# eromero-vlc/superbblas

Hardware: AMD Instinct MI355X
Metric: lattice contraction GFLOP/s + permute GB/s, 16^4 spin×color, 1/2/4/8 GPUs (higher is better)
Workload: dtype complex<f64>

## Files before the change

superbblas_amd/csrc/capi.cpp:

```cpp
#include "plan.h"
#include <atomic>
#include <algorithm>
#include <functional>
#include <memory>
#include <unordered_map>

#include <rccl/rccl.h>

#include <cstdlib>
#include <cstring>
#include <mutex>

namespace sbx {
BsrOp *bsr_create(int nd, int ni, int dtype, const std::vector<std::vector<Range>> &pi,
                  const Coor &dimi, const std::vector<std::vector<Range>> &pd, const Coor &dimd,
                  const Coor &blocki, const Coor &blockd, bool block_im_fast,
                  const std::vector<const int *> &ii, const std::vector<const int *> &jj,
                  const std::vector<const void *> &v, const std::vector<int> &devs, bool reverse_jj,
                  const Comm &comm, const Coor *kroni = nullptr, const Coor *krond = nullptr,
                  const std::vector<const void *> *kronv = nullptr);
void bsr_destroy(BsrOp *op);
void bsr_krylov(const BsrOp &op, const Scalar &alpha, const std::string &oi,
                const std::string &od, const DistTensor &x, const Coor &fromx, const Coor &sizex,
                const Scalar &beta, const DistTensor &y, const Coor &fromy, const Coor &sizey,
// ... 304 lines not shown
        tapes().clear();
    });
}

int sbx_clear_handles(void) {
    return guard([&] {
        trim_pools();
        destroy_streams();
    });
}

int sbx_allocate(unsigned long long bytes, sbx_context ctx, void **ptr) {
    return guard([&] {
        if (ctx.plat == SBX_GPU) {
            *ptr = device_alloc(bytes, ctx.device);
        } else {
            SBX_HIP_CHECK(hipHostMalloc(ptr, bytes, hipHostMallocDefault));
        }
    });
}

int sbx_deallocate(void *ptr, sbx_context ctx) {
    return guard([&] {
        if (!ptr) return;
        if (ctx.plat == SBX_GPU) {
            set_device(ctx.device);
            SBX_HIP_CHECK(hipStreamSynchronize(get_stream(ctx.device)));
            device_free(ptr, ctx.device);
        } else {
            SBX_HIP_CHECK(hipHostFree(ptr));
        }
    });
}

int sbx_set_custom_allocator(sbx_alloc_fn alloc, sbx_free_fn dealloc, void *user) {
    return guard([&] {
        if ((alloc == nullptr) != (dealloc == nullptr))
            throw Error("set_custom_allocator: give both functions or neither");
        set_alloc_hooks(alloc, dealloc, user);
    });
}

int sbx_allocate_from_cache(unsigned long long bytes, sbx_context ctx, void **ptr) {
    return guard([&] {
        if (ctx.plat != SBX_GPU) throw Error("allocate_from_cache: GPU contexts only");
        *ptr = scratch_alloc(bytes, ctx.device);
    });
}

int sbx_release_to_cache(void *ptr, sbx_context ctx) {
    return guard([&] {
        if (ctx.plat != SBX_GPU) throw Error("release_to_cache: GPU contexts only");
        scratch_free(ptr, ctx.device);
    });
}

int sbx_cache_usage(int device, unsigned long long *cached, unsigned long long *live) {
    return guard([&] {
        std::size_t c = 0, l = 0;
        cache_usage(device, &c, &l);
        if (cached) *cached = c;
        if (live) *live = l;
    });
}

int sbx_tune_set(const char *key, long long value) {
    return guard([&] {
        if (!key) throw Error("tune_set: null key");
        const std::string k(key);
        if (k == "copy.budget") g_copy_tune.budget = (long)value;
        else if (k == "copy.run") g_copy_tune.run = (long)value;
        else if (k == "copy.nt") g_copy_tune.nt = (int)value;
        else if (k == "copy.max_elems") g_copy_tune.max_elems = (long)value;
        else if (k == "copy.pair") g_copy_tune.pair = (int)value;
        else if (k == "copy.order") g_copy_tune.order = (int)value;
        else if (k == "copy.trans") g_copy_tune.trans = (int)value;
        else if (k == "copy.btrans") g_copy_tune.btrans = (int)value;
        else if (k == "gemm.max_bytes") g_gemm_tune.max_bytes = (long)value;
        else if (k == "gemm.loaders") g_gemm_tune.loaders = (int)value;
        else if (k == "gemm.dma_spread") g_gemm_tune.dma_spread = (int)value;
        else if (k == "gemm.dma_nt") g_gemm_tune.dma_nt = (int)value;
        else if (k == "gemm.lean") g_gemm_tune.lean = (int)value;
        else if (k == "gemm.skinny") g_gemm_tune.skinny = (int)value;
        else if (k == "bsr.variant") g_bsr_tune.variant = (int)value;
        else if (k == "bsr.row_max_cols") g_bsr_tune.row_max_cols = (long)value;
        else if (k == "bsr.split_max_cols") g_bsr_tune.split_max_cols = (long)value;
        else if (k == "bsr.split_cw") g_bsr_tune.split_cw = (int)value;
        else if (k == "bsr.split_jb") g_bsr_tune.split_jb = (int)value;
        else if (k == "bsr.split_ilv") g_bsr_tune.split_ilv = (int)value;
        else if (k == "bsr.kron_mfma") g_bsr_tune.kron_mfma = (int)value;
        else if (k == "bsr.kron_mfma_min_cols") g_bsr_tune.kron_mfma_min_cols = (long)value;
        else if (k == "bsr.kron_pack") g_bsr_tune.kron_pack = (int)value;
        else if (k == "bsr.kron_xlds") g_bsr_tune.kron_xlds = (int)value;
        else if (k == "bsr.kron_ylds") g_bsr_tune.kron_ylds = (int)value;
        else if (k == "bsr.kron_spin") g_bsr_tune.kron_spin = (int)value;
        else if (k == "bsr.kron_adj") g_bsr_tune.kron_adj = (int)value;
        else if (k == "bsr.kron_spin_min_cols") g_bsr_tune.kron_spin_min_cols = (long)value;
        else if (k == "bsr.kron_order") g_bsr_tune.kron_order = (int)value;
        else if (k == "bsr.nt") g_bsr_tune.nt = (int)value;
        else if (k == "dense.wave") g_dense_wave = (int)value;
        else if (k == "bsr.blk_pd") g_bsr_tune.blk_pd = (int)value;
        else if (k == "bsr.blk_mfma") g_bsr_tune.blk_mfma = (int)value;
        else if (k == "bsr.blk_min") g_bsr_tune.blk_min = (int)value;
        else if (k == "bsr.mixed") g_bsr_tune.mixed = (int)value;
        else if (k == "bsr.mixed12_min_cols") g_bsr_tune.mixed12_min_cols = (long)value;
        else if (k == "bsr.mixed12_pack") g_bsr_tune.mixed12_pack = (int)value;
        else if (k == "bsr.adj_inplace") g_bsr_tune.adj_inplace = (int)value;
        else if (k == "bsr.kron_mixed") g_bsr_tune.kron_mixed = (int)value;
        else if (k == "bsr.adj_copy_bytes") throw Error("tune_set: bsr.adj_copy_bytes is read-only");
        else if (k == "bsr.tile") g_bsr_tune.tile = (int)value;
        else if (k == "bsr.tile_min_cols") g_bsr_tune.tile_min_cols = value;
        else if (k == "gemm.m3") g_gemm_tune.m3 = (int)value;
        else if (k == "gemm.splits") g_gemm_tune.splits = (int)value;
        else if (k == "gemm.t48") g_gemm_tune.t48 = (int)value;
        else if (k == "gemm.share_ab") g_gemm_tune.share_ab = (int)value;
        else if (k == "gemm.herm") g_gemm_tune.herm = (int)value;
        else if (k == "gemm.frag") g_gemm_tune.frag = (int)value;
        else if (k == "gemm.dot_wgs") g_gemm_tune.dot_wgs = (int)value;
        else if (k == "gemm.frag_tall") g_gemm_tune.frag_tall = (int)value;
        else if (k == "gemm.frag_pair") g_gemm_tune.frag_pair = (int)value;
        else if (k == "gemm.frag_nt") g_gemm_tune.frag_nt = (int)value;
        else if (k == "gemm.frag_small") g_gemm_tune.frag_small = (int)value;
        else if (k == "gemm.frag_uk") g_gemm_tune.frag_uk = (int)value;
        else if (k == "gemm.frag_waves") g_gemm_tune.frag_waves = (int)value;
        else if (k == "gemm.clock") {
            g_gemm_tune.clock = (int)value;
            unsigned long long v[3];
            gemm_clock_read(current_device(), v, true);
        }
        else if (k == "dist.reduce") g_dist_reduce = (int)value;
        else if (k == "debug.level") g_debug_level = (int)value;
        else if (k == "debug.corrupt_copy") g_debug_corrupt = (int)value;
        else if (k == "dist.reduce_calls") g_dist_reduce_calls = value;
        else if (k == "dist.force_peer") g_dist_force_peer = (int)value;
        else if (k == "dist.peer_copies") g_dist_peer_copies = value;
        else if (k.compare(0, 6, "alloc.") == 0) alloc_tune(key, nullptr, &value);
        else throw Error("tune_set: unknown key " + k);
        if (k.compare(0, 5, "copy.") == 0) {
            std::lock_guard<std::mutex> g(g_tape_mutex);
            tapes().clear();
        }
    });
}

int sbx_tune_get(const char *key, long long *value) {
    return guard([&] {
        if (!key || !value) throw Error("tune_get: null argument");
        const std::string k(key);
        if (k == "copy.budget") *value = g_copy_tune.budget;
        else if (k == "copy.run") *value = g_copy_tune.run;
        else if (k == "copy.nt") *value = g_copy_tune.nt;
        else if (k == "copy.max_elems") *value = g_copy_tune.max_elems;
        else if (k == "copy.pair") *value = g_copy_tune.pair;
        else if (k == "copy.order") *value = g_copy_tune.order;
        else if (k == "copy.trans") *value = g_copy_tune.trans;
        else if (k == "copy.btrans") *value = g_copy_tune.btrans;
        else if (k == "copy.last_pair") *value = g_copy_tune.last_pair;
        else if (k == "gemm.max_bytes") *value = g_gemm_tune.max_bytes;
        else if (k == "gemm.loaders") *value = g_gemm_tune.loaders;
        else if (k == "gemm.dma_spread") *value = g_gemm_tune.dma_spread;
        else if (k == "gemm.dma_nt") *value = g_gemm_tune.dma_nt;
        else if (k == "gemm.lean") *value = g_gemm_tune.lean;
        else if (k == "gemm.last_lean") *value = g_gemm_tune.last_lean;
        else if (k == "gemm.skinny") *value = g_gemm_tune.skinny;
        else if (k == "bsr.variant") *value = g_bsr_tune.variant;
        else if (k == "bsr.row_max_cols") *value = g_bsr_tune.row_max_cols;
        else if (k == "bsr.split_max_cols") *value = g_bsr_tune.split_max_cols;
        else if (k == "bsr.split_cw") *value = g_bsr_tune.split_cw;
        else if (k == "bsr.split_jb") *value = g_bsr_tune.split_jb;
        else if (k == "bsr.split_ilv") *value = g_bsr_tune.split_ilv;
        else if (k == "bsr.kron_mfma") *value = g_bsr_tune.kron_mfma;
        else if (k == "bsr.kron_mfma_min_cols") *value = g_bsr_tune.kron_mfma_min_cols;
        else if (k == "bsr.kron_pack") *value = g_bsr_tune.kron_pack;
        else if (k == "bsr.kron_xlds") *value = g_bsr_tune.kron_xlds;
        else if (k == "bsr.kron_ylds") *value = g_bsr_tune.kron_ylds;
        else if (k == "bsr.kron_spin") *value = g_bsr_tune.kron_spin;
        else if (k == "bsr.kron_adj") *value = g_bsr_tune.kron_adj;
        else if (k == "bsr.kron_spin_min_cols") *value = g_bsr_tune.kron_spin_min_cols;
        else if (k == "bsr.kron_order") *value = g_bsr_tune.kron_order;
        else if (k == "bsr.nt") *value = g_bsr_tune.nt;
        else if (k == "dense.wave") *value = g_dense_wave;
        else if (k == "bsr.blk_pd") *value = g_bsr_tune.blk_pd;
        else if (k == "bsr.blk_mfma") *value = g_bsr_tune.blk_mfma;
        else if (k == "bsr.blk_min") *value = g_bsr_tune.blk_min;
        else if (k == "bsr.tile") *value = g_bsr_tune.tile;
        else if (k == "bsr.tile_min_cols") *value = g_bsr_tune.tile_min_cols;
        else if (k == "bsr.mixed") *value = g_bsr_tune.mixed;
        else if (k == "bsr.mixed12_min_cols") *value = g_bsr_tune.mixed12_min_cols;
        else if (k == "bsr.mixed12_pack") *value = g_bsr_tune.mixed12_pack;
        else if (k == "bsr.last_kernel") *value = g_bsr_tune.last;
        else if (k == "bsr.last_mixed") *value = g_bsr_tune.last_mixed;
        else if (k == "bsr.adj_inplace") *value = g_bsr_tune.adj_inplace;
        else if (k == "bsr.kron_mixed") *value = g_bsr_tune.kron_mixed;
        else if (k == "bsr.adj_copy_bytes") *value = g_bsr_tune.adj_copy_bytes;
        else if (k == "gemm.m3") *value = g_gemm_tune.m3;
        else if (k == "gemm.splits") *value = g_gemm_tune.splits;
        else if (k == "gemm.t48") *value = g_gemm_tune.t48;
        else if (k == "gemm.share_ab") *value = g_gemm_tune.share_ab;
        else if (k == "gemm.herm") *value = g_gemm_tune.herm;
        else if (k == "gemm.last_herm") *value = g_gemm_tune.last_herm;
        else if (k == "gemm.frag") *value = g_gemm_tune.frag;
        else if (k == "gemm.dot_wgs") *value = g_gemm_tune.dot_wgs;
        else if (k == "gemm.frag_tall") *value = g_gemm_tune.frag_tall;
        else if (k == "gemm.frag_pair") *value = g_gemm_tune.frag_pair;
        else if (k == "gemm.frag_nt") *value = g_gemm_tune.frag_nt;
        else if (k == "gemm.frag_small") *value = g_gemm_tune.frag_small;
        else if (k == "gemm.frag_uk") *value = g_gemm_tune.frag_uk;
        else if (k == "gemm.frag_waves") *value = g_gemm_tune.frag_waves;
        else if (k == "gemm.clock") *value = g_gemm_tune.clock;
        else if (k == "gemm.clock_cycles" || k == "gemm.clock_ticks" || k == "gemm.clock_launches") {
            unsigned long long v[3];
            gemm_clock_read(current_device(), v, false);
            *value = (long long)v[k == "gemm.clock_cycles" ? 0 : k == "gemm.clock_ticks" ? 1 : 2];
        }
        else if (k == "dist.reduce") *value = g_dist_reduce;
        else if (k == "debug.level") *value = g_debug_level;
        else if (k == "debug.corrupt_copy") *value = g_debug_corrupt;
        else if (k == "dist.reduce_calls") *value = g_dist_reduce_calls;
        else if (k == "dist.force_peer") *value = g_dist_force_peer;
        else if (k == "dist.peer_copies") *value = g_dist_peer_copies;
        else if (k == "detail.last_device") *value = g_detail_last_device;
        else if (k.compare(0, 6, "alloc.") == 0) alloc_tune(key, value, nullptr);
        else throw Error("tune_get: unknown key " + k);
    });
}

int sbx_timings_enable(int on) {
    return guard([&] { timings_enable(on != 0); });
}

int sbx_timings_filter(const char *names) {
    return guard([&] { timings_filter(names && *names ? names : nullptr); });
}

int sbx_timings_reset(void) {
    return guard([&] { timings_reset(); });
}

int sbx_timings_get(const char *name, double *ms, long long *calls) {
    return guard([&] {
        if (!name || !ms || !calls) throw Error("timings_get: null argument");
        timings_get(name, ms, calls);
    });
}

int sbx_timings_report(char *buf, int len) {
    return guard([&] {
// ... 1023 lines not shown
```

superbblas_amd/csrc/kernels_gemm.hip:

```cpp
#include "sbx_internal.h"

#include <algorithm>
#include <map>
#include <mutex>
#include <cstdint>
#include <type_traits>

namespace sbx {
GemmTune g_gemm_tune;
namespace {

template <typename R> struct Mfma;
template <> struct Mfma<double> {
    typedef double acc_t __attribute__((ext_vector_type(4)));
    static __device__ __forceinline__ acc_t mma(double a, double b, acc_t c) {
        return __builtin_amdgcn_mfma_f64_16x16x4f64(a, b, c, 0, 0, 0);
    }
    static __device__ __forceinline__ int row(int lane, int r) { return (lane >> 4) + 4 * r; }
};
template <> struct Mfma<float> {
    typedef float acc_t __attribute__((ext_vector_type(4)));
    static __device__ __forceinline__ acc_t mma(float a, float b, acc_t c) {
        return __builtin_amdgcn_mfma_f32_16x16x4f32(a, b, c, 0, 0, 0);
    }
    static __device__ __forceinline__ int row(int lane, int r) { return ((lane >> 4) << 2) + r; }
};

template <typename R, bool CPLX> struct Elem;
template <> struct Elem<double, true> { typedef double2 type; };
template <> struct Elem<double, false> { typedef double type; };
template <> struct Elem<float, true> { typedef float2 type; };
template <> struct Elem<float, false> { typedef float type; };

template <typename E> __device__ __forceinline__ E zero_elem() { return E{}; }
[[maybe_unused]] __device__ __forceinline__ double2 conj_if(double2 v, bool c) { return c ? double2{v.x, -v.y} : v; }
__device__ __forceinline__ float2 conj_if(float2 v, bool c) { return c ? float2{v.x, -v.y} : v; }
__device__ __forceinline__ double conj_if(double v, bool) { return v; }
__device__ __forceinline__ float conj_if(float v, bool) { return v; }

template <typename E> __device__ __forceinline__ E buf_load(__amdgpu_buffer_rsrc_t r, unsigned off);
template <> [[maybe_unused]] __device__ __forceinline__ double2 buf_load<double2>(__amdgpu_buffer_rsrc_t r, unsigned off) {
    auto v = __builtin_amdgcn_raw_buffer_load_b128(r, off, 0, 0);
    return __builtin_bit_cast(double2, v);
}
template <> __device__ __forceinline__ double buf_load<double>(__amdgpu_buffer_rsrc_t r, unsigned off) {
    auto v = __builtin_amdgcn_raw_buffer_load_b64(r, off, 0, 0);
    return __builtin_bit_cast(double, v);
}
template <> __device__ __forceinline__ float2 buf_load<float2>(__amdgpu_buffer_rsrc_t r, unsigned off) {
    auto v = __builtin_amdgcn_raw_buffer_load_b64(r, off, 0, 0);
    return __builtin_bit_cast(float2, v);
}
template <> __device__ __forceinline__ float buf_load<float>(__amdgpu_buffer_rsrc_t r, unsigned off) {
    auto v = __builtin_amdgcn_raw_buffer_load_b32(r, off, 0, 0);
    return __builtin_bit_cast(float, v);
}

struct GemmKArgs {
    long m, n, k, batch;
    const void *a;
    long sa_m, sa_k, sa_b;
    const void *b;
    long sb_k, sb_n, sb_b;
    void *c;
    long sc_m, sc_n, sc_b;
    double alpha_re, alpha_im, beta_re, beta_im;
    int conja, conjb;
    int splits;
    int herm;
    long kchunk;
    void *work;
    unsigned long long *probe;
    int probe_all;
    int tm, tn;
    unsigned a_bytes, b_bytes;
    int split;
    long m_lo, n_lo, k_lo;
    long sa_m_hi, sa_k_hi, sb_k_hi, sb_n_hi, sc_m_hi, sc_n_hi;
    int same_ab;
    int dma_nt;
    int pair_a, pair_b;
};

__device__ __forceinline__ long split_off(long i, long lo, long s, long s_hi) {
    const unsigned q = (unsigned)i / (unsigned)lo;
    return (long)q * s_hi + (long)((unsigned)i - q * (unsigned)lo) * s;
}
__device__ __forceinline__ long c_off(const GemmKArgs &p, long gi, long gj) {
    return p.split ? split_off(gi, p.m_lo, p.sc_m, p.sc_m_hi) + split_off(gj, p.n_lo, p.sc_n, p.sc_n_hi)
                   : gi * p.sc_m + gj * p.sc_n;
}

template <typename R>
__device__ __forceinline__ void epilogue_store(R *cptr, R vr, R vi, const GemmKArgs &p, bool cplx) {
    if (cplx) {
        R ar = (R)p.alpha_re, ai = (R)p.alpha_im;
        R outr = ar * vr - ai * vi, outi = ar * vi + ai * vr;
        if (p.beta_re != 0 || p.beta_im != 0) {
            R br = (R)p.beta_re, bi = (R)p.beta_im;
            R cr = cptr[0], ci = cptr[1];
            outr += br * cr - bi * ci;
            outi += br * ci + bi * cr;
        }
        cptr[0] = outr;
        cptr[1] = outi;
    } else {
        R out = (R)p.alpha_re * vr;
        if (p.beta_re != 0) out += (R)p.beta_re * cptr[0];
        cptr[0] = out;
    }
}


__device__ __forceinline__ int xcd_workgroup() {
    const int nwg = gridDim.x, bid = blockIdx.x;
    const int xcd = bid & 7, q = nwg >> 3, rr = nwg & 7;
    return (xcd < rr ? xcd * (q + 1) : rr * (q + 1) + (xcd - rr) * q) + (bid >> 3);
}

struct KRange {
    long begin, end;
};
__device__ __forceinline__ KRange split_k_range(const GemmKArgs &p, int split) {
    const long k_begin = (long)split * p.kchunk;
    return KRange{k_begin, min(p.k, k_begin + p.kchunk)};
}

struct Tile {
    int ti, tj, split;
    long bb, m0, n0, k_begin, k_end;
    __device__ __forceinline__ void finish(const GemmKArgs &p, int rest, int BM, int BN) {
        split = rest % p.splits;
        bb = rest / p.splits;
        m0 = (long)ti * BM, n0 = (long)tj * BN;
        const KRange kr = split_k_range(p, split);
        k_begin = kr.begin, k_end = kr.end;
    }
};
__device__ __forceinline__ Tile tile_of(const GemmKArgs &p, int wg, int BM, int BN) {
    Tile t;
    t.ti = wg % p.tm;
    int rest = wg / p.tm;
    t.tj = rest % p.tn;
    t.finish(p, rest / p.tn, BM, BN);
    return t;
}
__device__ __forceinline__ Tile upper_tile_of(const GemmKArgs &p, int wg, int BM) {
    Tile t;
    const long ntri = (long)p.tm * (p.tm + 1) / 2;
    const long tt = wg % ntri;
    long c = (long)((__fsqrt_rn(8.f * (float)tt + 1.f) - 1.f) * 0.5f);
    while (c * (c + 1) / 2 > tt) --c;
    while ((c + 1) * (c + 2) / 2 <= tt) ++c;
    t.tj = (int)c;
    t.ti = (int)(tt - c * (c + 1) / 2);
    t.finish(p, (int)(wg / ntri), BM, BM);
    return t;
}

template <typename E>
__device__ __forceinline__ __amdgpu_buffer_rsrc_t operand_rsrc(const void *base, long bb, long s_b,
                                                               unsigned bytes) {
    return __builtin_amdgcn_make_buffer_rsrc((void *)((const E *)base + bb * s_b), (short)0,
                                             (int)bytes, 0x00020000);
}

template <typename R> struct ConjMask {
    typedef typename std::conditional<sizeof(R) == 8, unsigned long long, unsigned>::type U;
    U ma, mb;
    __device__ __forceinline__ ConjMask(const GemmKArgs &p) {
        const U sign = (U)1 << (sizeof(R) * 8 - 1);
        ma = p.conja ? sign : 0, mb = p.conjb ? sign : 0;
    }
    static __device__ __forceinline__ R flip(R v, U m) {
        return __builtin_bit_cast(R, __builtin_bit_cast(U, v) ^ m);
    }
    template <typename E, int MT, int NT>
    __device__ __forceinline__ void apply(E (&af)[MT], E (&bf)[NT]) const {
#pragma unroll
        for (int i = 0; i < MT; ++i) af[i].y = flip(af[i].y, ma);
#pragma unroll
        for (int j = 0; j < NT; ++j) bf[j].y = flip(bf[j].y, mb);
    }
};

template <typename A, int MT, int NT, typename... More>
__device__ __forceinline__ void zero_acc(A (&acc)[MT][NT], More &...more) {
#pragma unroll
    for (int i = 0; i < MT; ++i)
#pragma unroll
        for (int j = 0; j < NT; ++j) {
            acc[i][j] = A{0, 0, 0, 0};
// ... 975 lines not shown
    const KRange kr = split_k_range(p, split);
    const long k0 = kr.begin, k1 = kr.end;
    const E *A = (const E *)p.a + bb * p.sa_b, *B = (const E *)p.b + bb * p.sb_b;
    const int m = (int)p.m, n = (int)p.n;
    E acc[MM][NN];
#pragma unroll
    for (int i = 0; i < MM; ++i)
#pragma unroll
        for (int j = 0; j < NN; ++j) acc[i][j] = zero_elem<E>();
    constexpr int U = 4;
    for (long k = k0 + threadIdx.x; k < k1; k += 256 * U) {
        E a[U][MM], b[U][NN];
#pragma unroll
        for (int u = 0; u < U; ++u) {
            const long kk = k + 256L * u;
            const bool in = kk < k1;
#pragma unroll
            for (int i = 0; i < MM; ++i)
                a[u][i] = in && i < m ? conj_if(A[i * p.sa_m + kk * p.sa_k], p.conja) : zero_elem<E>();
#pragma unroll
            for (int j = 0; j < NN; ++j)
                b[u][j] = in && j < n ? conj_if(B[kk * p.sb_k + j * p.sb_n], p.conjb) : zero_elem<E>();
        }
#pragma unroll
        for (int u = 0; u < U; ++u)
#pragma unroll
            for (int i = 0; i < MM; ++i)
#pragma unroll
                for (int j = 0; j < NN; ++j) acc[i][j] = madd(acc[i][j], a[u][i], b[u][j]);
    }
    __shared__ E red[4][MM * NN];
    const int lane = threadIdx.x & 63, wave = threadIdx.x >> 6;
#pragma unroll
    for (int i = 0; i < MM; ++i)
#pragma unroll
        for (int j = 0; j < NN; ++j) {
            E v = acc[i][j];
#pragma unroll
            for (int o = 32; o >= 1; o >>= 1) v = xor_sum(v, o);
            if (lane == 0) red[wave][i * NN + j] = v;
        }
    __syncthreads();
    const int t = threadIdx.x;
    if (t < m * n) {
        const int i = t % m, j = t / m;
        E v = red[0][i * NN + j];
#pragma unroll
        for (int w = 1; w < 4; ++w) {
            if constexpr (CPLX) {
                v.x += red[w][i * NN + j].x;
                v.y += red[w][i * NN + j].y;
            } else {
                v += red[w][i * NN + j];
            }
        }
        if (p.splits == 1)
            store_out<R, CPLX>(p, bb, i, j, v);
        else
            ((E *)p.work)[(((long)split * p.batch + bb) * p.n + j) * p.m + i] = v;
    }
}

template <typename R, bool CPLX, int NN>
__global__ void __launch_bounds__(256) gemm_rows_kernel(const GemmKArgs p) {
    typedef typename Elem<R, CPLX>::type E;
    const long total = p.m * p.batch;
    const int n = (int)p.n;
    for (long idx = blockIdx.x * 256L + threadIdx.x; idx < total; idx += (long)gridDim.x * 256L) {
        const long i = idx % p.m, bb = idx / p.m;
        const E *A = (const E *)p.a + bb * p.sa_b + i * p.sa_m;
        const E *B = (const E *)p.b + bb * p.sb_b;
        E acc[NN];
#pragma unroll
        for (int j = 0; j < NN; ++j) acc[j] = zero_elem<E>();
        for (long k = 0; k < p.k; ++k) {
            const E a = conj_if(A[k * p.sa_k], p.conja);
#pragma unroll
            for (int j = 0; j < NN; ++j)
                if (j < n) acc[j] = madd(acc[j], a, conj_if(B[k * p.sb_k + j * p.sb_n], p.conjb));
        }
#pragma unroll
        for (int j = 0; j < NN; ++j)
            if (j < n) store_out<R, CPLX>(p, bb, i, j, acc[j]);
    }
}

template <typename R, bool CPLX, int UK, bool KP = false, int NT = 1>
__global__ void __launch_bounds__(256) gemm_frag_kernel(const GemmKArgs p) {
    typedef typename Elem<R, CPLX>::type E;
    typedef typename Mfma<R>::acc_t acc_t;
    constexpr int ES = (int)sizeof(E);
    const int lane = threadIdx.x & 63;
    const long item = (long)blockIdx.x * 4 + (threadIdx.x >> 6);
    const long items = (long)p.tm * p.tn * p.batch * p.splits;
    if (item >= items) return;
    const int split = (int)(item % p.splits);
    long rest = item / p.splits;
    const long ti = rest % p.tm;
    rest /= p.tm;
    const long tj = rest % p.tn;
    const long bb = rest / p.tn;
    const long m0 = ti * 16, n0 = tj * 16 * NT;
    const long k_begin = (long)split * p.kchunk, k_end = min(p.k, k_begin + p.kchunk);
    const __amdgpu_buffer_rsrc_t rsA = operand_rsrc<E>(p.a, bb, p.sa_b, p.a_bytes);
    const __amdgpu_buffer_rsrc_t rsB = operand_rsrc<E>(p.b, bb, p.sb_b, p.b_bytes);
    const int r = lane & 15, q = lane >> 4;
    const bool okA = m0 + r < p.m;
    const long baseA = (m0 + r) * p.sa_m;
    bool okB[NT];
    long baseB[NT];
#pragma unroll
    for (int j = 0; j < NT; ++j) {
        okB[j] = n0 + 16 * j + r < p.n;
        baseB[j] = (n0 + 16 * j + r) * p.sb_n;
    }
    const ConjMask<R> cj(p);
    static_assert(!KP || (ES == 8 && UK % 2 == 0), "k pairs: 8-byte elements, even UK");
    auto load = [&](long k0, E (&a)[UK], E (&b)[NT][UK]) {
        if constexpr (KP) {
#pragma unroll
            for (int u = 0; u < UK; u += 2) {
                const long kk = k0 + 4 * u + 2 * q;
                const bool kin = kk < k_end;
                auto pair = [&](__amdgpu_buffer_rsrc_t rs, bool ok, bool paired, long base, long sk,
                                E &lo, E &hi) {
                    if (paired) {
                        const auto v = __builtin_amdgcn_raw_buffer_load_b128(
                            rs, ok && kin ? (unsigned)((base + kk) * ES) : 0x80000000u, 0, 0);
                        typedef typename std::conditional<sizeof(R) == 8, double, float2>::type H;
                        struct Two { H lo, hi; };
                        const Two t = __builtin_bit_cast(Two, v);
                        lo = __builtin_bit_cast(E, t.lo);
                        hi = __builtin_bit_cast(E, t.hi);
                    } else {
                        lo = buf_load<E>(rs, ok && kin ? (unsigned)((base + kk * sk) * ES) : 0x80000000u);
                        hi = buf_load<E>(rs, ok && kin ? (unsigned)((base + (kk + 1) * sk) * ES) : 0x80000000u);
                    }
                };
                pair(rsA, okA, p.pair_a != 0, baseA, p.sa_k, a[u], a[u + 1]);
#pragma unroll
                for (int j = 0; j < NT; ++j)
                    pair(rsB, okB[j], p.pair_b != 0, baseB[j], p.sb_k, b[j][u], b[j][u + 1]);
            }
        } else {
#pragma unroll
            for (int u = 0; u < UK; ++u) {
                const long kk = k0 + 4 * u + q;
                const bool kin = kk < k_end;
                a[u] = buf_load<E>(rsA, okA && kin ? (unsigned)((baseA + kk * p.sa_k) * ES) : 0x80000000u);
#pragma unroll
                for (int j = 0; j < NT; ++j)
                    b[j][u] = buf_load<E>(rsB, okB[j] && kin ? (unsigned)((baseB[j] + kk * p.sb_k) * ES) : 0x80000000u);
            }
        }
    };
    acc_t accR[NT], accI[NT];
#pragma unroll
    for (int j = 0; j < NT; ++j) {
        accR[j] = acc_t{0, 0, 0, 0};
        accI[j] = acc_t{0, 0, 0, 0};
    }
    E a[UK], b[NT][UK], an[UK], bn[NT][UK];
    if (k_begin < k_end) load(k_begin, a, b);
    for (long k = k_begin; k < k_end; k += 4 * UK) {
        if (k + 4 * UK < k_end) load(k + 4 * UK, an, bn);
#pragma unroll
// ... 361 lines not shown
            } else
                launch_dma_cfg<R, CPLX, AK, BK, 128, 128, 16, 4, 4, false, false, 1, false, 0, 1, HM>(p, device, stream, 0, 256);
        } else {
            launch_dma_cfg<R, CPLX, AK, BK, 64, 64, 8, 2, 2, true, false, 1, false, 0, 1, HM>(p, device, stream, 0, 1024);
        }
    } else {
        const int t48 = g_gemm_tune.t48;
        if (t48 > 0 && p.m > 32 && p.m <= 48 && p.n > 32 && p.n <= 48) {
            if (t48 == 1) return launch_dma_cfg<R, CPLX, AK, BK, 48, 48, 16, 3, 1>(p, device, stream, 0, 1024);
            if (t48 == 2) return launch_dma_cfg<R, CPLX, AK, BK, 48, 48, 16, 1, 3>(p, device, stream, 0, 1024);
            if (t48 == 3) return launch_dma_cfg<R, CPLX, AK, BK, 48, 48, 32, 3, 1>(p, device, stream, 0, 1024);
            if (t48 == 4) return launch_dma_cfg<R, CPLX, AK, BK, 48, 48, 16, 3, 1>(p, device, stream, 0, 1536);
            const bool sh = g_gemm_tune.share_ab && same_operands(p);
            if constexpr (!AK && !BK && sizeof(E) >= 8) {
                if (sh && t48 == 13) return launch_wave_cfg<R, CPLX, AK, 48, 8, 4, 2>(p, device, stream, 1024);
                if (sh && t48 == 14) return launch_wave_cfg<R, CPLX, AK, 48, 16, 4, 2>(p, device, stream, 768);
                if (sh && t48 == 16) return launch_wave_cfg<R, CPLX, AK, 48, 8, 16, 2>(p, device, stream, 256);
                if (sh && t48 == 17) return launch_wave_cfg<R, CPLX, AK, 48, 8, 8, 2, true>(p, device, stream, 512);
                if (sh && t48 != 6) return launch_wave_cfg<R, CPLX, AK, 48, 8, 8, 2>(p, device, stream, 512);
            }
            return launch_dma_cfg<R, CPLX, AK, BK, 48, 48, 32, 1, 1, false, false, 4>(p, device, stream, 0, 768);
        }
        if (p.m >= 128 && p.n >= 128)
            launch_dma_cfg<R, CPLX, AK, BK, 128, 128, 32, 4, 2, true, false, 1, false, 0, 1, HM>(p, device, stream, 0, 256);
        else
            launch_dma_cfg<R, CPLX, AK, BK, 64, 64, 32, 2, 2, true, false, 1, false, 0, 1, HM>(p, device, stream, 0, 1024);
    }
}

template <typename R, bool CPLX> bool launch_skinny(const GemmKArgs &p0, int device, hipStream_t s) {
    if (!g_gemm_tune.skinny || p0.split) return false;
    typedef typename Elem<R, CPLX>::type E;
    GemmKArgs p = p0;
    if (p.m <= 4 && p.n <= 4) {
        const long wgs = std::max(1, g_gemm_tune.dot_wgs);
        long splits = std::max(1L, std::min((wgs + p.batch - 1) / p.batch, (p.k + 1023) / 1024));
        p.kchunk = (p.k + splits - 1) / splits;
        splits = std::max(1L, (p.k + p.kchunk - 1) / p.kchunk);
        p.splits = (int)splits;
        Scratch work;
        if (splits > 1) {
            work = Scratch(sizeof(E) * splits * p.batch * p.m * p.n, device);
            p.work = work.ptr;
        }
        const long nwg = p.batch * splits;
        if (nwg > 0x7fffffffL) return false;
        timed_launch<R, CPLX>(p, s, [&] {
            const long mx = std::max(p.m, p.n);
            if (mx == 1)
                hipLaunchKernelGGL((gemm_dot_kernel<R, CPLX, 1, 1>), dim3((unsigned)nwg), dim3(256), 0, s, p);
            else if (mx == 2)
                hipLaunchKernelGGL((gemm_dot_kernel<R, CPLX, 2, 2>), dim3((unsigned)nwg), dim3(256), 0, s, p);
            else
                hipLaunchKernelGGL((gemm_dot_kernel<R, CPLX, 4, 4>), dim3((unsigned)nwg), dim3(256), 0, s, p);
        });
        return true;
    }
    const bool rows = p.n <= 16 && p.m >= 2 * p.n && p.k <= 64;
    const bool cols = p.m <= 16 && p.n >= 2 * p.m && p.k <= 64;
    if (!rows && !cols) return false;
    if (!rows) {
        std::swap(p.m, p.n);
        std::swap(p.a, p.b);
        std::swap(p.sa_m, p.sb_n);
        std::swap(p.sa_k, p.sb_k);
        std::swap(p.sa_b, p.sb_b);
        std::swap(p.conja, p.conjb);
        std::swap(p.sc_m, p.sc_n);
    }
    const long total = p.m * p.batch;
    const long blocks = std::max(1L, std::min((total + 255) / 256, 65536L));
    timed_launch<R, CPLX>(p, s, [&] {
        if (p.n == 1)
            hipLaunchKernelGGL((gemm_rows_kernel<R, CPLX, 1>), dim3((unsigned)blocks), dim3(256), 0, s, p);
        else if (p.n <= 2)
            hipLaunchKernelGGL((gemm_rows_kernel<R, CPLX, 2>), dim3((unsigned)blocks), dim3(256), 0, s, p);
        else if (p.n <= 4)
            hipLaunchKernelGGL((gemm_rows_kernel<R, CPLX, 4>), dim3((unsigned)blocks), dim3(256), 0, s, p);
        else if (p.n <= 8)
            hipLaunchKernelGGL((gemm_rows_kernel<R, CPLX, 8>), dim3((unsigned)blocks), dim3(256), 0, s, p);
        else
            hipLaunchKernelGGL((gemm_rows_kernel<R, CPLX, 16>), dim3((unsigned)blocks), dim3(256), 0, s, p);
    });
    return true;
}

template <typename R, bool CPLX> bool launch_frag(const GemmKArgs &p0, int device, hipStream_t s) {
    if (!g_gemm_tune.frag || p0.split || (CPLX && g_gemm_tune.m3 > 0)) return false;
    const long sm = g_gemm_tune.frag_small;
    const bool small = p0.m <= sm && p0.n <= sm;
    typedef typename Elem<R, CPLX>::type E;
    const long tn = g_gemm_tune.frag_tall > 0 ? g_gemm_tune.frag_tall
                    : (CPLX && sizeof(R) == 4) ? 48 : 16;
    const bool tall = (p0.n <= 16 && p0.n > 4 && p0.m <= 16) ||
                      (p0.n <= tn && p0.n > 4 && p0.k <= 64 && p0.k > 4) ||
                      (p0.m <= tn && p0.m > 4 && p0.k <= 64 && p0.k > 4);
    if (!small && !tall) return false;
    if (g_gemm_tune.skinny && p0.m <= 4 && p0.n <= 4 && g_gemm_tune.frag < 2) return false;
    const int auto_uk = p0.k <= 8 || (p0.m <= 32 && p0.n <= 32) ? 2 : 4;
    const int uk = g_gemm_tune.frag_uk == 0 ? auto_uk : g_gemm_tune.frag_uk == 8 ? 8
                 : g_gemm_tune.frag_uk == 2 ? 2 : 4;
    const int nt = g_gemm_tune.frag_nt == 4 ? 4 : g_gemm_tune.frag_nt == 2 ? 2
                 : g_gemm_tune.frag_nt == 0 && small && p0.n > 16 ? 2 : 1;
    GemmKArgs p = p0;
    Scratch work;
    const long items = prepare_launch<E>(p, 16, 16 * nt, 4 * uk, 0,
                                         std::max(64, g_gemm_tune.frag_waves), work, device);
    const long blocks = (items + 3) / 4;
    if (blocks > 0x7fffffffL) return false;
    auto aligned = [](const void *ptr, long s1, long s2) {
        return ((std::uintptr_t)ptr % 16) == 0 && s1 % 2 == 0 && s2 % 2 == 0;
    };
    constexpr bool E8 = sizeof(E) == 8;
    p.pair_a = E8 && p.sa_k == 1 && aligned(p.a, p.sa_m, p.sa_b);
    p.pair_b = E8 && p.sb_k == 1 && aligned(p.b, p.sb_n, p.sb_b);
    const bool kp = E8 && g_gemm_tune.frag_pair && p.k % 2 == 0 &&
                    (p.pair_a || (p.pair_b && p.n > 16));
    timed_launch<R, CPLX>(p, s, [&] {
        const dim3 grid((unsigned)blocks), wg(256);
        auto go = [&](auto ukc, auto kpc, auto ntc) {
            constexpr int UKv = decltype(ukc)::value, NTv = decltype(ntc)::value;
            constexpr bool KPv = decltype(kpc)::value;
            hipLaunchKernelGGL((gemm_frag_kernel<R, CPLX, UKv, KPv, NTv>), grid, wg, 0, s, p);
        };
        auto by_nt = [&](auto ukc, auto kpc) {
            if (nt == 4)
                go(ukc, kpc, std::integral_constant<int, 4>());
            else if (nt == 2)
                go(ukc, kpc, std::integral_constant<int, 2>());
            else
                go(ukc, kpc, std::integral_constant<int, 1>());
        };
        auto by_uk = [&](auto kpc) {
            if (uk == 8)
                by_nt(std::integral_constant<int, 8>(), kpc);
            else if (uk == 2)
                by_nt(std::integral_constant<int, 2>(), kpc);
            else
                by_nt(std::integral_constant<int, 4>(), kpc);
        };
        if constexpr (E8) {
            if (kp) by_uk(std::true_type());
        }
        if (!kp) by_uk(std::false_type());
    });
    return true;
}

template <typename R, bool CPLX> void launch_typed(const GemmKArgs &p, int device, hipStream_t s) {
    if (launch_frag<R, CPLX>(p, device, s)) return;
    if (launch_skinny<R, CPLX>(p, device, s)) return;
    const bool ak = (p.sa_k == 1) || (p.sa_m != 1 && std::labs(p.sa_k) <= std::labs(p.sa_m));
    const bool bk = (p.sb_k == 1) || (p.sb_n != 1 && std::labs(p.sb_k) <= std::labs(p.sb_n));
    if (ak && bk)
        launch_tiled<R, CPLX, true, true>(p, device, s);
    else if (ak && !bk)
        launch_tiled<R, CPLX, true, false>(p, device, s);
    else if (!ak && bk)
        launch_tiled<R, CPLX, false, true>(p, device, s);
    else
        launch_tiled<R, CPLX, false, false>(p, device, s);
}

template <typename R, bool CPLX> void launch_scale(const GemmKArgs &p, hipStream_t s) {
    const long total = p.batch * p.m * p.n;
    if (total == 0) return;
    const long blocks = std::min((total + 255) / 256, 4096L);
    hipLaunchKernelGGL((scale_c_kernel<R, CPLX>), dim3((unsigned)blocks), dim3(256), 0, s, p);
    SBX_HIP_CHECK(hipGetLastError());
}

GemmKArgs make_args(const GemmDesc &d) {
    GemmKArgs p{};
    p.m = d.m;
    p.n = d.n;
    p.k = d.k;
    p.batch = d.batch;
    p.a = d.a;
    p.sa_m = d.sa_m;
    p.sa_k = d.sa_k;
    p.sa_b = d.sa_b;
    p.b = d.b;
    p.sb_k = d.sb_k;
    p.sb_n = d.sb_n;
    p.sb_b = d.sb_b;
    p.c = d.c;
    p.sc_m = d.sc_m;
    p.sc_n = d.sc_n;
    p.sc_b = d.sc_b;
    p.alpha_re = d.alpha.re;
    p.alpha_im = dtype_is_complex(d.t) ? d.alpha.im : 0;
    p.beta_re = d.beta.re;
    p.beta_im = dtype_is_complex(d.t) ? d.beta.im : 0;
    p.conja = d.conja;
    p.conjb = d.conjb;
    p.splits = 1;
    p.kchunk = d.k;
    p.m_lo = d.m_lo > 0 ? d.m_lo : d.m;
    p.n_lo = d.n_lo > 0 ? d.n_lo : d.n;
    p.k_lo = d.k_lo > 0 ? d.k_lo : d.k;
    p.sa_m_hi = d.sa_m_hi;
    p.sa_k_hi = d.sa_k_hi;
    p.sb_k_hi = d.sb_k_hi;
    p.sb_n_hi = d.sb_n_hi;
    p.sc_m_hi = d.sc_m_hi;
    p.sc_n_hi = d.sc_n_hi;
    p.split = (p.m_lo != p.m || p.n_lo != p.n || p.k_lo != p.k) ? 1 : 0;
    if (p.split && (p.m_lo < 1 || p.n_lo < 1 || p.k_lo < 1 || p.m % p.m_lo || p.n % p.n_lo ||
                    p.k % p.k_lo))
        throw Error("gemm: invalid split groups");
    return p;
}

template <typename P1, typename P2>
void bisect_gemm(const GemmDesc &d, int device, long GemmDesc::*n, long GemmDesc::*lo,
                 P1 GemmDesc::*p1, long s1, long s1_hi, P2 GemmDesc::*p2, long s2, long s2_hi,
                 bool accumulate) {
    const bool groups = d.*lo > 0 && d.*lo < d.*n;
    const long o = groups ? d.*n / d.*lo / 2 : d.*n / 2;
    const long n1 = groups ? o * d.*lo : o;
    const long es = (long)dtype_size(d.t);
    GemmDesc a = d, b = d;
    a.*n = n1;
    b.*n = d.*n - n1;
    a.*lo = b.*lo = groups ? d.*lo : 0;
    b.*p1 = (P1)((const char *)(d.*p1) + es * o * (groups ? s1_hi : s1));
    b.*p2 = (P2)((const char *)(d.*p2) + es * o * (groups ? s2_hi : s2));
    if (accumulate) b.beta = Scalar{1, 0};
    launch_gemm(a, device);
    launch_gemm(b, device);
}

}

void gemm_clock_read(int device, unsigned long long out[3], bool reset) {
    clock_read_impl(device, out, reset);
}

void launch_gemm(const GemmDesc &d, int device) {
    if (d.m == 0 || d.n == 0 || d.batch == 0) return;
    if (d.k > 0 && (d.alpha.re != 0 || d.alpha.im != 0)) {
        const long es = (long)dtype_size(d.t);
        const long max_bytes = g_gemm_tune.max_bytes > 0 ? g_gemm_tune.max_bytes : (1L << 31) - 1;
        const long ea = (group_extent(d.m, d.m_lo, d.sa_m, d.sa_m_hi) +
                         group_extent(d.k, d.k_lo, d.sa_k, d.sa_k_hi) + 1) * es;
        const long eb = (group_extent(d.k, d.k_lo, d.sb_k, d.sb_k_hi) +
                         group_extent(d.n, d.n_lo, d.sb_n, d.sb_n_hi) + 1) * es;
        if (ea > max_bytes || eb > max_bytes) {
            if (d.k > 1)
                return bisect_gemm(d, device, &GemmDesc::k, &GemmDesc::k_lo, &GemmDesc::a, d.sa_k,
                                   d.sa_k_hi, &GemmDesc::b, d.sb_k, d.sb_k_hi, true);
            if (d.m > 1 && (ea > max_bytes || d.n <= 1))
                return bisect_gemm(d, device, &GemmDesc::m, &GemmDesc::m_lo, &GemmDesc::a, d.sa_m,
                                   d.sa_m_hi, &GemmDesc::c, d.sc_m, d.sc_m_hi, false);
            if (d.n > 1)
                return bisect_gemm(d, device, &GemmDesc::n, &GemmDesc::n_lo, &GemmDesc::b, d.sb_n,
                                   d.sb_n_hi, &GemmDesc::c, d.sc_n, d.sc_n_hi, false);
            throw Error("gemm: operand batch entries of 2 GiB or more are not supported");
        }
    }
    set_device(device);
    hipStream_t s = get_stream(device);
    GemmKArgs p = make_args(d);
    g_gemm_tune.last_herm = 0;
    g_gemm_tune.last_lean = 0;
    const bool scale_only = (d.k == 0 || (p.alpha_re == 0 && p.alpha_im == 0));
    switch (d.t) {
    case SBX_CDOUBLE:
        scale_only ? launch_scale<double, true>(p, s) : launch_typed<double, true>(p, device, s);
        break;
    case SBX_DOUBLE:
        scale_only ? launch_scale<double, false>(p, s) : launch_typed<double, false>(p, device, s);
        break;
    case SBX_CFLOAT:
        scale_only ? launch_scale<float, true>(p, s) : launch_typed<float, true>(p, device, s);
        break;
    case SBX_FLOAT:
        scale_only ? launch_scale<float, false>(p, s) : launch_typed<float, false>(p, device, s);
        break;
    default: throw Error("gemm: unsupported type");
    }
}

}
```

superbblas_amd/csrc/sbx_internal.h:

```cpp
#pragma once

#include <hip/hip_runtime.h>

#include <array>
#include <atomic>
#include <complex>
#include <cstdint>
#include <cstring>
#include <memory>
#include <stdexcept>
#include <string>
#include <vector>

#include "../../include/superbblas_amd/sbx.h"

namespace sbx {

struct Error : public std::runtime_error {
    explicit Error(const std::string &s) : std::runtime_error(s) {}
};

#define SBX_HIP_CHECK(expr)                                                                        \
    do {                                                                                           \
        hipError_t sbx_e_ = (expr);                                                                \
// ... 82 lines not shown
struct KernelTimer {
    const char *name;
    hipStream_t stream;
    void *ev0 = nullptr;
    KernelTimer(const char *name, hipStream_t s);
    ~KernelTimer();
};


struct GemmDesc {
    int t;
    long m, n, k, batch;
    const void *a;
    long sa_m, sa_k, sa_b;
    bool conja;
    const void *b;
    long sb_k, sb_n, sb_b;
    bool conjb;
    void *c;
    long sc_m, sc_n, sc_b;
    Scalar alpha, beta;
    long m_lo = 0, n_lo = 0, k_lo = 0;
    long sa_m_hi = 0, sa_k_hi = 0, sb_k_hi = 0, sb_n_hi = 0, sc_m_hi = 0, sc_n_hi = 0;
};
void launch_gemm(const GemmDesc &d, int device);

struct BoxCopyDesc {
    int src_t, dst_t;
    const void *src;
    void *dst;
    std::vector<long> size, src_stride, dst_stride;
    Scalar alpha;
    bool add;
    const float *src_mask = nullptr, *dst_mask = nullptr;
};
void launch_box_copy(const BoxCopyDesc &d, int device);
void clear_copy_launch_cache();
int copy_kernel_plan(const BoxCopyDesc &d, long *blocks);

struct TapeLaunch {
    std::shared_ptr<const void> launch;
    const void *src;
    void *dst;
    int device;
    Scalar alpha;
    int src_arg = -1, src_comp = -1, dst_arg = -1, dst_comp = -1;
    long src_off = 0, dst_off = 0;
    bool alpha_is_call = false;
};
struct CopyTape {
    std::vector<TapeLaunch> launches;
    bool valid = true;
};
void set_copy_tape(CopyTape *t);
CopyTape *current_copy_tape();
void replay_launch(const TapeLaunch &l, const void *src, void *dst, const Scalar &alpha);
void clear_copy_plan_cache();
struct CopyTune {
    long budget = 0;
    long run = 0;
    int nt = 0;
    long max_elems = 0;
    int pair = 0;
    int order = 0;
    int trans = 0;
    int btrans = 0;
    std::atomic<int> last_pair{0};
};
extern CopyTune g_copy_tune;
struct GemmTune {
    int m3 = 0;
    int splits = 0;
    long max_bytes = 0;
    int t48 = 5;
    int share_ab = 1;
    int herm = 0;
    std::atomic<int> last_herm{0};
    int loaders = 8;
    int dma_spread = 1;
    int dma_nt = 0;
    int lean = 1;
    std::atomic<int> last_lean{0};
    int skinny = 1;
    int clock = 0;
    int dot_wgs = 256;
    int frag_uk = 0;
    int frag_waves = 4096;
    int frag = 1;
    int frag_small = 32;
    int frag_nt = 0;
    int frag_pair = 1;
    int frag_tall = 0;
};
uint32_t storage_checksum(const void *p, std::size_t bytes, std::size_t blocksize, uint32_t prev);
void gemm_clock_read(int device, unsigned long long out[3], bool reset);
extern GemmTune g_gemm_tune;
struct BsrTune {
    int variant = 0;
    long row_max_cols = 3;
    long split_max_cols = 32;
    int split_cw = 0;
    int split_jb = 0;
    int split_ilv = 2;
    int kron_mfma = 1;
    long kron_mfma_min_cols = 8;
    int kron_pack = 1;
    int kron_xlds = 1;
    int kron_ylds = 0;
    int kron_spin = 0;
    long kron_spin_min_cols = 8;
    int kron_order = 1;
    int kron_adj = 1;
    int blk_pd = 1;
    int tile = 0;
    long tile_min_cols = 33;
    int nt = 11;
    int blk_mfma = 1;
    int blk_min = 16;
    int mixed = 1;
    long mixed12_min_cols = 4;
    int mixed12_pack = 1;
    int adj_inplace = 0;
    int kron_mixed = 0;
    std::atomic<long long> adj_copy_bytes{0};
    std::atomic<int> last{0};
    std::atomic<int> last_mixed{0};
};
extern BsrTune g_bsr_tune;
extern int g_dense_wave;

inline void check_dma_lds(const char *kernel, size_t lds, long passes, long lanes_per_pass,
                   long extra_bytes = 0) {
    const long need = passes * lanes_per_pass * 16 + extra_bytes;
    if ((long)lds < need)
        throw Error(std::string("bsr: internal LDS sizing error in ") + kernel + ": " +
                    std::to_string(lds) + " bytes for DMA passes needing " + std::to_string(need));
}

void launch_zero(void *p, std::size_t bytes, int device);

struct IndexCopyDesc {
    int src_t, dst_t;
    const void *src;
    void *dst;
    const int *src_idx = nullptr, *dst_idx = nullptr;
    long n = 0, blocking = 1;
    Scalar alpha;
    bool add = false;
};
void launch_index_copy(const IndexCopyDesc &d, int device);

struct TileSched {
    const int *rows = nullptr, *uniq = nullptr;
    const unsigned char *loc = nullptr;
    int umax = 0, tt = 0;
    long chunks = 0;
};

struct BsrDesc {
    int t;
    int tv;
    long block_rows;
    int bi, bd;
    const int *ii;
    const int *jj;
    const void *v;
// ... 38 lines not shown
```

Measured before the change: 73660.

## Add streaming row-GEMM kernel for tall-skinny shapes with nontemporal loads/stores

Adds a new GEMM path for tall-skinny complex/real products (small n and k, unit-stride m). Each workgroup processes a persistent range of 256-row tiles, stages the small B matrix in LDS once per batch, keeps a full row of A in registers, and writes C with optional nontemporal stores and loads once the working set exceeds 256 MiB. The aim is to make these bandwidth-bound contractions stream memory better than the existing frag/skinny kernels. Because it is enabled by default and placed ahead of the other paths, it may displace tuned kernels for some shapes.

```diff
diff --git a/superbblas_amd/csrc/capi.cpp b/superbblas_amd/csrc/capi.cpp
--- a/superbblas_amd/csrc/capi.cpp
+++ b/superbblas_amd/csrc/capi.cpp
@@ -410,6 +410,9 @@
         else if (k == "gemm.dma_nt") g_gemm_tune.dma_nt = (int)value;
         else if (k == "gemm.lean") g_gemm_tune.lean = (int)value;
         else if (k == "gemm.skinny") g_gemm_tune.skinny = (int)value;
+        else if (k == "gemm.rows_stream") g_gemm_tune.rows_stream = (int)value;
+        else if (k == "gemm.rows_stream_wgs") g_gemm_tune.rows_stream_wgs = (int)value;
+        else if (k == "gemm.rows_stream_nt") g_gemm_tune.rows_stream_nt = (int)value;
         else if (k == "bsr.variant") g_bsr_tune.variant = (int)value;
         else if (k == "bsr.row_max_cols") g_bsr_tune.row_max_cols = (long)value;
         else if (k == "bsr.split_max_cols") g_bsr_tune.split_max_cols = (long)value;
@@ -491,6 +494,10 @@
         else if (k == "gemm.lean") *value = g_gemm_tune.lean;
         else if (k == "gemm.last_lean") *value = g_gemm_tune.last_lean;
         else if (k == "gemm.skinny") *value = g_gemm_tune.skinny;
+        else if (k == "gemm.rows_stream") *value = g_gemm_tune.rows_stream;
+        else if (k == "gemm.rows_stream_wgs") *value = g_gemm_tune.rows_stream_wgs;
+        else if (k == "gemm.rows_stream_nt") *value = g_gemm_tune.rows_stream_nt;
+        else if (k == "gemm.last_rows_stream") *value = g_gemm_tune.last_rows_stream;
         else if (k == "bsr.variant") *value = g_bsr_tune.variant;
         else if (k == "bsr.row_max_cols") *value = g_bsr_tune.row_max_cols;
         else if (k == "bsr.split_max_cols") *value = g_bsr_tune.split_max_cols;
diff --git a/superbblas_amd/csrc/kernels_gemm.hip b/superbblas_amd/csrc/kernels_gemm.hip
--- a/superbblas_amd/csrc/kernels_gemm.hip
+++ b/superbblas_amd/csrc/kernels_gemm.hip
@@ -91,7 +91,7 @@
                    : gi * p.sc_m + gj * p.sc_n;
 }
 
-template <typename R>
+template <typename R, bool NT = false>
 __device__ __forceinline__ void epilogue_store(R *cptr, R vr, R vi, const GemmKArgs &p, bool cplx) {
     if (cplx) {
         R ar = (R)p.alpha_re, ai = (R)p.alpha_im;
@@ -102,12 +102,20 @@
             outr += br * cr - bi * ci;
             outi += br * ci + bi * cr;
         }
-        cptr[0] = outr;
-        cptr[1] = outi;
+        if constexpr (NT) {
+            typedef R v2 __attribute__((ext_vector_type(2)));
+            __builtin_nontemporal_store(v2{outr, outi}, (v2 *)cptr);
+        } else {
+            cptr[0] = outr;
+            cptr[1] = outi;
+        }
     } else {
         R out = (R)p.alpha_re * vr;
         if (p.beta_re != 0) out += (R)p.beta_re * cptr[0];
-        cptr[0] = out;
+        if constexpr (NT)
+            __builtin_nontemporal_store(out, cptr);
+        else
+            cptr[0] = out;
     }
 }
 
@@ -1249,6 +1257,90 @@
 #pragma unroll
         for (int j = 0; j < NN; ++j)
             if (j < n) store_out<R, CPLX>(p, bb, i, j, acc[j]);
+    }
+}
+
+template <typename E, bool NT>
+__device__ __forceinline__ E buf_load_policy(__amdgpu_buffer_rsrc_t r, unsigned off) {
+    constexpr int AUX = NT ? 2 : 0;
+    if constexpr (sizeof(E) == 16)
+        return __builtin_bit_cast(E, __builtin_amdgcn_raw_buffer_load_b128(r, off, 0, AUX));
+    else if constexpr (sizeof(E) == 8)
+        return __builtin_bit_cast(E, __builtin_amdgcn_raw_buffer_load_b64(r, off, 0, AUX));
+    else
+        return __builtin_bit_cast(E, __builtin_amdgcn_raw_buffer_load_b32(r, off, 0, AUX));
+}
+
+template <typename R, bool CPLX, int KK, bool NT>
+__global__ void __launch_bounds__(256) gemm_rows_stream_kernel(const GemmKArgs p) {
+    typedef typename Elem<R, CPLX>::type E;
+    constexpr int ES = (int)sizeof(E);
+    constexpr int NN = 16, JB = 4;
+    __shared__ E Bs[KK * NN];
+    const int n = (int)p.n, kn = (int)p.k;
+    const long blocks_m = p.tm;
+    const long units = blocks_m * p.batch;
+    const long per = (units + gridDim.x - 1) / gridDim.x;
+    const long u0 = blockIdx.x * per, u1 = min(units, u0 + per);
+    long staged = -1;
+    for (long u = u0; u < u1; ++u) {
+        const long bb = u / blocks_m;
+        const long i = (u - bb * blocks_m) * 256 + threadIdx.x;
+        const bool ok = i < p.m;
+        const __amdgpu_buffer_rsrc_t rsA = operand_rsrc<E>(p.a, bb, p.sa_b, p.a_bytes);
+        E a[KK];
+#pragma unroll
+        for (int k = 0; k < KK; ++k)
+            a[k] = buf_load_policy<E, NT>(rsA, ok && k < kn ? (unsigned)((i + k * p.sa_k) * ES) : 0x80000000u);
+        if (bb != staged) {
+            if (staged >= 0) __syncthreads();
+            const E *B = (const E *)p.b + bb * p.sb_b;
+            for (int t = threadIdx.x; t < KK * NN; t += 256) {
+                const int k = t / NN, j = t % NN;
+                Bs[t] = k < kn && j < n ? conj_if(B[k * p.sb_k + j * p.sb_n], p.conjb) : zero_elem<E>();
+            }
+            __syncthreads();
+            staged = bb;
+        }
+#pragma unroll
+        for (int k = 0; k < KK; ++k) a[k] = conj_if(a[k], p.conja);
+        R *c = (R *)c_ptr<E, false>(p, bb, i, 0);
+        for (int j0 = 0; j0 < n; j0 += JB) {
+            E acc[JB];
+#pragma unroll
+            for (int j = 0; j < JB; ++j) acc[j] = zero_elem<E>();
+            E b[JB], bn[JB];
+#pragma unroll
+            for (int j = 0; j < JB; ++j) b[j] = Bs[j0 + j];
+#pragma unroll
+            for (int k = 0; k < KK; ++k) {
+                if (k + 1 < KK) {
+#pragma unroll
+                    for (int j = 0; j < JB; ++j) bn[j] = Bs[(k + 1) * NN + j0 + j];
+                }
+#pragma unroll
+                for (int j = 0; j < JB; ++j) acc[j] = madd(acc[j], a[k], b[j]);
+                __builtin_amdgcn_sched_barrier(0);
+#pragma unroll
+                for (int j = 0; j < JB; ++j) b[j] = bn[j];
+            }
+#pragma unroll
+            for (int j = 0; j < JB; ++j) {
+                if constexpr (CPLX)
+                    asm volatile("" : "+v"(acc[j].x), "+v"(acc[j].y));
+                else
+                    asm volatile("" : "+v"(acc[j]));
+            }
+#pragma unroll
+            for (int j = 0; j < JB; ++j) {
+                if (!ok || j0 + j >= n) continue;
+                R *cptr = c + (j0 + j) * p.sc_n * (CPLX ? 2 : 1);
+                if constexpr (CPLX)
+                    epilogue_store<R, NT>(cptr, acc[j].x, acc[j].y, p, true);
+                else
+                    epilogue_store<R, NT>(cptr, acc[j], R(0), p, false);
+            }
+        }
     }
 }
 
@@ -1776,6 +1868,54 @@
         else
             hipLaunchKernelGGL((gemm_rows_kernel<R, CPLX, 16>), dim3((unsigned)blocks), dim3(256), 0, s, p);
     });
+    return true;
+}
+
+template <typename R, bool CPLX> bool launch_rows_stream(const GemmKArgs &p0, int device, hipStream_t s) {
+    if (g_gemm_tune.rows_stream <= 0 || !g_gemm_tune.skinny || p0.split || p0.k > 16) return false;
+    if (p0.sa_k < 0 || p0.sa_m < 0 || p0.sb_k < 0 || p0.sb_n < 0) return false;
+    const bool rows = p0.n <= 16 && p0.m > 16 && p0.m >= 2 * p0.n && p0.sa_m == 1 && p0.sc_m == 1;
+    const bool cols = p0.m <= 16 && p0.n > 16 && p0.n >= 2 * p0.m && p0.sb_n == 1 && p0.sc_n == 1;
+    if (!rows && !cols) return false;
+    typedef typename Elem<R, CPLX>::type E;
+    const long tiny = std::max(std::min(p0.m, p0.n), p0.k);
+    const long tiny_min = !CPLX && sizeof(R) == 4 ? 4 : 3;
+    if (tiny < tiny_min && g_gemm_tune.rows_stream < 2) return false;
+    GemmKArgs p = p0;
+    if (!rows) {
+        std::swap(p.m, p.n);
+        std::swap(p.m_lo, p.n_lo);
+        std::swap(p.a, p.b);
+        std::swap(p.sa_m, p.sb_n);
+        std::swap(p.sa_k, p.sb_k);
+        std::swap(p.sa_b, p.sb_b);
+        std::swap(p.conja, p.conjb);
+        std::swap(p.sc_m, p.sc_n);
+    }
+    Scratch work;
+    const long units = prepare_launch<E>(p, 256, 16, 1, 1, 0, work, device);
+    const long wgs = g_gemm_tune.rows_stream_wgs > 0 ? g_gemm_tune.rows_stream_wgs : 8192;
+    const dim3 grid((unsigned)std::max(1L, std::min(units, wgs))), wg(256);
+    const long bytes = (long)sizeof(E) * p.batch * p.m * (p.k + p.n);
+    const bool nt = g_gemm_tune.rows_stream_nt > 0 || (g_gemm_tune.rows_stream_nt == 0 && bytes > (256L << 20));
+    timed_launch<R, CPLX>(p, s, [&] {
+        auto go = [&](auto kkc) {
+            constexpr int KKv = decltype(kkc)::value;
+            if (nt)
+                hipLaunchKernelGGL((gemm_rows_stream_kernel<R, CPLX, KKv, true>), grid, wg, 0, s, p);
+            else
+                hipLaunchKernelGGL((gemm_rows_stream_kernel<R, CPLX, KKv, false>), grid, wg, 0, s, p);
+        };
+        if (p.k <= 4)
+            go(std::integral_constant<int, 4>());
+        else if (p.k <= 8)
+            go(std::integral_constant<int, 8>());
+        else if (p.k <= 12)
+            go(std::integral_constant<int, 12>());
+        else
+            go(std::integral_constant<int, 16>());
+    });
+    g_gemm_tune.last_rows_stream = 1;
     return true;
 }
 
@@ -1842,6 +1982,7 @@
 }
 
 template <typename R, bool CPLX> void launch_typed(const GemmKArgs &p, int device, hipStream_t s) {
+    if (launch_rows_stream<R, CPLX>(p, device, s)) return;
     if (launch_frag<R, CPLX>(p, device, s)) return;
     if (launch_skinny<R, CPLX>(p, device, s)) return;
     const bool ak = (p.sa_k == 1) || (p.sa_m != 1 && std::labs(p.sa_k) <= std::labs(p.sa_m));
@@ -1958,6 +2099,7 @@
     GemmKArgs p = make_args(d);
     g_gemm_tune.last_herm = 0;
     g_gemm_tune.last_lean = 0;
+    g_gemm_tune.last_rows_stream = 0;
     const bool scale_only = (d.k == 0 || (p.alpha_re == 0 && p.alpha_im == 0));
     switch (d.t) {
     case SBX_CDOUBLE:
diff --git a/superbblas_amd/csrc/sbx_internal.h b/superbblas_amd/csrc/sbx_internal.h
--- a/superbblas_amd/csrc/sbx_internal.h
+++ b/superbblas_amd/csrc/sbx_internal.h
@@ -188,6 +188,10 @@
     int lean = 1;
     std::atomic<int> last_lean{0};
     int skinny = 1;
+    int rows_stream = 1;
+    int rows_stream_wgs = 0;
+    int rows_stream_nt = 0;
+    std::atomic<int> last_rows_stream{0};
     int clock = 0;
     int dot_wgs = 256;
     int frag_uk = 0;
```

Result: no change. 73630 (median of 2 runs) (-0.0%).
